# HKUST-KnowComp/DummyNode4GraphLearning

Measured on AMD Instinct MI355X. Metric: edges/sec fwd+bwd on dummy-augmented RGIN conv, higher is better.
Workload: dtype bf16; 1 GPU; config5: RGINLayer(256,256,R=16,basis,relu) fwd+bwd, ONE global batch of 32768 graphs cut by parallel.shard_graphs over 1 GPU(s) (rank 0: N=1015808, E=3997696), SI dummy augmentation; global_edges=3997696, parallelism=dp1, rows_P=3112960, grad_bucket_bytes=2491904, hip_graph=True, sub_batches=1

## Files before the change

### dummynode4graphlearning_amd/_lib.py

```python
import ctypes
import os

import torch

_HERE = os.path.dirname(os.path.abspath(__file__))
LIB_PATH = os.environ.get("DN_HIP_LIB") or os.path.join(_HERE, "libdn_hip.so")

c_i32, c_i64, c_f32, c_sz = ctypes.c_int32, ctypes.c_int64, ctypes.c_float, ctypes.c_size_t
P = ctypes.c_void_p

class WgradJob(ctypes.Structure):
    _fields_ = [("A", P), ("A2", P), ("idx_a", P), ("G", P), ("G2", P), ("idx_g", P), ("mask_a_bits", P), ("na1", c_i32), ("ng1", c_i32),
                ("colsum_of", c_i32), ("first_rel", c_i32), ("row0", c_i32), ("act_slope", c_f32)]


_SIGS = {
    "dn_version": (ctypes.c_int, []),
    "dn_last_error": (ctypes.c_char_p, []),
    "dn_runtime_probe": (ctypes.c_int, [P]),
    "dn_gather_segsum_f32": (ctypes.c_int, [P, c_i64, c_i32, P, P, P, c_i64, c_i64, P, P, c_f32, c_i32, P]),
    "dn_gather_segsum_bf16": (ctypes.c_int, [P, c_i64, c_i32, P, P, P, c_i64, c_i64, P, P, c_f32, c_i32, P]),
    "dn_segment_sum_f32": (ctypes.c_int, [P, c_i32, P, c_i64, P, P]),
    "dn_segment_sum_bf16": (ctypes.c_int, [P, c_i32, P, c_i64, P, P]),
    "dn_segment_mean_f32": (ctypes.c_int, [P, c_i32, P, c_i64, P, P]),
# ... 25 lines not shown
    "dn_row_index_workspace_bytes": (c_sz, [c_i64, c_i64, c_i64]),
    "dn_row_index_build_i32": (ctypes.c_int, [c_i64, c_i64, c_i64, P, P, P, c_i32, c_f32] + [P] * 10 +
                               [ctypes.POINTER(c_i64), ctypes.POINTER(c_i32), ctypes.POINTER(c_i32), P, c_sz, P]),
    "dn_row_index_local_workspace_bytes": (c_sz, [c_i64, c_i64, c_i64, c_i64]),
    "dn_row_index_build_local_i32": (ctypes.c_int, [c_i64, c_i64, c_i64, c_i64, P, P, P, P, P, c_i32, c_f32] + [P] * 10 +
                                     [ctypes.POINTER(c_i64), ctypes.POINTER(c_i32), ctypes.POINTER(c_i32),
                                      ctypes.POINTER(c_i32), P, P, P, P, P, ctypes.POINTER(c_i32), P, c_sz, P]),
    "dn_rows_wgrad_multi_bf16": (ctypes.c_int, [ctypes.POINTER(WgradJob), c_i32, c_i32, c_i64, P, c_i64, P, P, c_i32, P, P, P, c_sz, P]),
    "dn_rows_wgrad_multi_f32": (ctypes.c_int, [ctypes.POINTER(WgradJob), c_i32, c_i32, c_i64, P, c_i64, P, P, P, P, c_sz, P]),
    "dn_rows_chain2_f32": (ctypes.c_int, [P, c_i32, P, P, c_i32, P, P, P, P, c_i32, c_i64, P, P, c_i32, c_f32, P, P, P]),
    "dn_layer_graphs_fwd_bf16": (ctypes.c_int, [P, c_i32, P, P, P, c_i32, P, P, P, P, c_f32, P, P, P, P, P, c_i64, c_i64, P, P, P, P, P, P, P,
                                                P, P, P]),
    "dn_layer_graphs_bwd_bf16": (ctypes.c_int, [P, c_i32, P, P, c_i32, P, P, c_f32, P, P, P, P, P, P, P, c_i64, c_i64, P, P, P, P, P, P, P,
                                                P]),
    "dn_conv_graphs_max_nodes": (c_i32, []),
    "dn_conv_graphs_max_edges": (c_i32, []),
    "dn_conv_graphs_bf16": (ctypes.c_int, [P, c_i32, P, c_i32, P, P, c_i32, P, P, P, P, P, c_i64, c_i64, P, P, P, P, P, P]),
    "dn_conv_index_workspace_bytes": (c_sz, [c_i64, c_i64, c_i64, c_i64, c_i32, c_i64]),
    "dn_conv_index_build_i32": (ctypes.c_int, [c_i64, c_i64, c_i64, c_i64, P, P, P, P, P, c_i32, c_f32] + [P] * 10 +
                                [ctypes.POINTER(c_i64), ctypes.POINTER(c_i32), ctypes.POINTER(c_i32),
                                 ctypes.POINTER(c_i32), P, P, P, P, P, ctypes.POINTER(c_i32)] +
                                [c_i32, c_i32, c_i64] + [P] * 8 + [c_i32, c_i64] + [P] * 8 + [c_i32, c_i32, P, P] + [c_i32, c_i32, c_i64, P, P] +
                                [ctypes.POINTER(c_i32), P, c_sz, P]),
    "dn_row_tables_build_i32": (ctypes.c_int, [c_i32, P, c_i32, c_i64, P, P, ctypes.c_uint64, P]),
    "dn_sweep_tables_build_i32": (ctypes.c_int, [c_i32, P, P, P, c_i64, c_i32, c_i32, ctypes.c_uint64, P, P, P]),
    "dn_slot_table_build_i32": (ctypes.c_int, [c_i64, c_i32, c_i32, P, P, c_i32, c_i32, P, P, P, P]),
    "dn_fold_tables_build_async_i32": (ctypes.c_int, [c_i64, c_i64, P, P, P, P, P, P, c_sz, P]),
    "dn_rows_wgrad_workspace_bytes": (c_sz, [c_i64, c_i32, c_i32]),
    "dn_rows_wgrad_bf16": (ctypes.c_int, [P, P, c_i32, P, P, P, c_i32, P, c_i32, c_i32, c_i64, P, c_i64, P, P, c_i32,
                                          c_i32, P, P, P, P, P, c_f32, P, c_sz, P]),
    "dn_rows_transform_bf16": (ctypes.c_int, [P, P, c_i32, P, c_i32, c_i32, P, P, c_i32, P, P, c_i64, P, c_i32, c_f32, P]),
    "dn_relu_bwd_bf16": (ctypes.c_int, [P, P, P, c_i64, c_f32, P]),
    "dn_rows_chain2_bf16": (ctypes.c_int, [P, c_i32, P, P, c_i32, P, P, P, P, c_i32, c_i64, P, P, P, P, c_i32, c_f32, P]),
    "dn_rows_selfsum_bf16": (ctypes.c_int, [P, c_i32, P, P, P, P, c_i32, P, c_i32, c_i64, P, P, P, c_i32, P, P, c_i32, c_i32, c_i32, P]),
    "dn_overflow_rows_add_bf16": (ctypes.c_int, [P, c_i32, P, c_i32, c_i64, P, P, c_i32, c_i32, c_i32, P, P]),
    "dn_close_units_capacity": (c_i64, [c_i64, c_i64, c_i32]),
    "dn_close_units_workspace_bytes": (c_sz, [c_i64, c_i32]),
    "dn_close_units_build_i32": (ctypes.c_int, [c_i64, c_i32, c_i32, P, c_i64, c_i32, c_i32, P, P, c_i64, c_i32, c_i32, P, P, P, c_i64, P,
                                                P, P, P, c_i32, P, c_sz, P]),
    "dn_fold_graph_tiles_build_i32": (ctypes.c_int, [c_i64, c_i64, P, P, P, P, P, P, P]),
    "dn_fold_graph_tiles_multi_capacity": (c_i64, [c_i64, c_i32]),
    "dn_fold_graph_tiles_multi_build_i32": (ctypes.c_int, [c_i64, c_i64, P, P, P, c_i32, P, P, P, P, c_i64, P, P]),
    "dn_rows_close_bf16": (ctypes.c_int, [P, c_i32, P, c_i32, P, P, P, P, c_i32, P, P, c_i64, P, P, P, P, P, P, P]),
    "dn_bdd_compose": (ctypes.c_int, [P, c_i64, c_i32, c_i32, c_i32, c_i32, P, P]),
    "dn_bdd_extract": (ctypes.c_int, [P, c_i64, c_i32, c_i32, c_i32, c_i32, P, P]),
    "dn_fold_tables_workspace_bytes": (c_sz, [c_i64]),
    "dn_fold_tables_build_i32": (ctypes.c_int, [c_i64, c_i64, P, P, P, P, ctypes.POINTER(ctypes.c_int32), P, c_sz, P]),
    "dn_fold_tail_bf16": (ctypes.c_int, [P, P, c_i64, c_i32, P, P, P, P, c_i32, P]),
    "dn_rows_transform_f32": (ctypes.c_int, [P, P, c_i32, P, c_i32, c_i32, P, P, c_i32, P, P, c_i64, P, c_i32, c_f32, P, c_i32, c_i32, c_i32, P]),
    "dn_rows_wgrad_f32": (ctypes.c_int, [P, P, c_i32, P, P, P, c_i32, P, c_i32, c_i32, c_i64, P, c_i64, P, P, c_i32, P, P, P,
                                         c_i32, c_f32, P, c_sz, P]),
    "dn_relu_bwd_f32": (ctypes.c_int, [P, P, P, c_i64, c_f32, P]),
    "dn_rows_gemm_f32": (ctypes.c_int, [P, P, P, c_i32, c_i32, c_i32, P, c_i64, P, P]),
    "dn_rows_gemm_bf16": (ctypes.c_int, [P, P, P, c_i32, c_i32, c_i32, P, c_i64, P, P]),
    "dn_rows_wgrad_any_workspace_bytes": (c_sz, [c_i64, c_i32, c_i32]),
    "dn_rows_wgrad_any_f32": (ctypes.c_int, [P, P, c_i32, c_i32, c_i64, P, c_i64, P, P, P, P, c_sz, P]),
    "dn_rows_wgrad_any_bf16": (ctypes.c_int, [P, P, c_i32, c_i32, c_i64, P, c_i64, P, P, P, P, c_sz, P]),
    "dn_batchnorm_rows_workspace_bytes": (c_sz, [c_i64, c_i32]),
    "dn_batchnorm_rows_f32": (ctypes.c_int, [P, c_i64, c_i32, P, P, c_f32, P, P, P, P, P, P, c_f32, c_i32, P, P, c_sz, P]),
    "dn_batchnorm_rows_bf16": (ctypes.c_int, [P, c_i64, c_i32, P, P, c_f32, P, P, P, P, P, P, c_f32, c_i32, P, P, c_sz, P]),
    "dn_batchnorm_rows_bwd_f32": (ctypes.c_int, [P, P, c_i64, c_i32, P, P, P, P, c_i32, P, P, P, P, c_sz, P]),
    "dn_batchnorm_rows_bwd_bf16": (ctypes.c_int, [P, P, c_i64, c_i32, P, P, P, P, c_i32, P, P, P, P, c_sz, P]),
    "dn_edge_norm_f32": (ctypes.c_int, [c_i32, c_i32, c_i64, c_i64] + [P] * 7 + [P]),
    "dn_degrees_i32": (ctypes.c_int, [c_i64, c_i64, P, P, P, P, P]),
    "dn_si_filter_meta_f32": (ctypes.c_int, [c_i64, P, P, P, c_i64, P, P, P, c_i64, c_i32, c_i32, c_i32, c_i32, P, P, P]),
    "dn_si_filter_meta_bf16": (ctypes.c_int, [c_i64, P, P, P, c_i64, P, P, P, c_i64, c_i32, c_i32, c_i32, c_i32, P, P, P]),
# ... 116 lines not shown
```

### dummynode4graphlearning_amd/csrc/build.py

```python
import hashlib
import os
import subprocess
import sys
from concurrent.futures import ThreadPoolExecutor

HERE = os.path.dirname(os.path.abspath(__file__))
PKG = os.path.dirname(HERE)
ROOT = os.path.dirname(PKG)
SOURCES = ["dn_runtime.hip", "dn_segment.hip", "dn_index.hip", "dn_index_local.hip", "dn_conv_index.hip", "dn_graphsum.hip", "dn_rel.hip", "dn_rel_ring.hip", "dn_close.hip", "dn_conv_graph.hip", "dn_chain2.hip", "dn_weights.hip", "dn_rel_f32.hip", "dn_gemm.hip", "dn_norm.hip", "dn_simodel.hip", "dn_dual.hip"]
HEADERS = ["dn_common.h", "dn_internal.h", os.path.join(ROOT, "include", "dn_hip.h")]
LIB = os.path.join(PKG, "libdn_hip.so")
OBJDIR = os.path.join(HERE, "_obj")
ARCH = "gfx950"
FLAGS = ["-O3", "-std=c++17", "-fPIC", "--offload-arch=" + ARCH, "-fno-gpu-rdc", "-Wno-unused-result",
         "-I" + os.path.join(ROOT, "include")]


def _hipcc():
    for c in (os.environ.get("HIPCC"), "/opt/rocm/bin/hipcc", "hipcc"):
        if c and (os.path.isabs(c) and os.path.exists(c) or not os.path.isabs(c)):
            return c
    raise RuntimeError("hipcc not found")


def _digest(paths):
    h = hashlib.sha256()
    for p in paths:
        with open(p, "rb") as f:
            h.update(f.read())
    h.update(" ".join(FLAGS).encode())
    return h.hexdigest()


def build(force=False, verbose=True, tuning=False):
    global FLAGS
    if (tuning or os.environ.get("DN_BUILD_TUNING") == "1") and "-DDN_TUNING_ENV" not in FLAGS:
        FLAGS = FLAGS + ["-DDN_TUNING_ENV"]
    for extra in os.environ.get("DN_BUILD_EXTRA", "").split():
        if extra not in FLAGS:
            FLAGS = FLAGS + [extra]
    srcs = [os.path.join(HERE, s) for s in SOURCES if os.path.exists(os.path.join(HERE, s))]
    hdrs = [h if os.path.isabs(h) else os.path.join(HERE, h) for h in HEADERS]
# ... 37 lines not shown
```

### dummynode4graphlearning_amd/csrc/dn_internal.h

```cpp
#pragma once
#include <hip/hip_runtime.h>
#include <stdint.h>

namespace dn_internal {

int launch_transform_ring256(const void* X, const void* X2, int32_t n1, const int32_t* idx, const void* Wn, const void* bias,
                             int32_t relu, int32_t nt_store, const void* mask_pos, const int32_t* tiles, int64_t num_tiles,
                             int64_t tiles_per_wg, void* Y, int32_t w_kn, float slope, hipStream_t st);

bool chain2_ring_supported(bool has_mask0, bool has_mask1, bool has_bits1, bool has_bits2);
int launch_chain2_ring256(const void* X, const void* W1n, const void* b1, const void* W2n, const void* b2, int32_t flags,
                          const void* mask0, const void* mask1, int64_t N, void* Y1, void* Y2, void* bits1, void* bits2,
                          float slope, hipStream_t st);

constexpr int kRilPlanWords = 14;

int ril_queue(int64_t G, int64_t N, int64_t R, int64_t E, const int32_t* node_ptr, const int32_t* edge_ptr, const int32_t* src,
              const int32_t* dst, const int32_t* etype, int32_t self_loop, float edge_frac, int32_t* row_in, int32_t* row_out,
              int32_t* aux_f_ptr, int32_t* aux_f_idx, int32_t* aux_b_ptr, int32_t* aux_b_idx, int32_t* dst_ptr, int32_t* dst_rows,
              int32_t* src_ptr, int32_t* src_rows, int32_t* rel_ptr_dev, int32_t* tile_ptr_f, int32_t* fold_info_f,
              int32_t* tile_ptr_b, int32_t* fold_info_b, bool verdicts, bool plan, void* workspace, size_t workspace_bytes,
              int32_t** meta_dev, hipStream_t st);
void ril_unpack(const int32_t* h_meta, int64_t R, int64_t* host_counts, int32_t* host_rel_ptr, int32_t* host_modes,
                int32_t* host_status, int32_t* host_absorb);

struct CloseUnitsDir {
    const int32_t *tile_ptr, *list_ptr, *list_rows;
    int32_t num_edge_rows, drop_beg, drop_end;
    const int32_t *drop_enable, *dyn;
    int32_t *unit_ptr, *units, *ent_row;
    uint32_t* ent_mask;
    const int32_t *chunk_tile = nullptr, *chunk_graph = nullptr;
    int32_t chunks_per_wg = 0;
    const int32_t* tile_ptr_alt = nullptr;
};
struct FoldMultiDir {
    const int32_t *seg_ptr, *seg_nodes, *add_idx;
    int32_t *chunk_tile, *chunk_graph, *tile_ptr, *fold_info, *dev_ok;
    const int32_t* gate;
};
int fold_multi_queue(int64_t N, int64_t num_segments, int nd, const FoldMultiDir* dirs, int32_t num_chunks, int64_t tile_capacity,
                     bool with_valid, hipStream_t st);
int close_units_queue(int64_t N, int32_t num_wg, int64_t num_tiles, int32_t agg_units, int32_t xcd_order, int64_t num_list_entries,
                      int64_t unit_capacity, int nd, const CloseUnitsDir* dirs, void* workspace, size_t workspace_bytes, hipStream_t st,
                      int32_t alt_order, int64_t alt_num_tiles);

// ... 6 lines not shown
```

### dummynode4graphlearning_amd/csrc/dn_rel.hip

```cpp
#include <cstdlib>

#include "dn_common.h"
#include "dn_internal.h"
#include "../../include/dn_hip.h"

namespace {

typedef __bf16 bf16_t;
typedef short short4v __attribute__((ext_vector_type(4)));
typedef short short8v __attribute__((ext_vector_type(8)));
typedef bf16_t bf16x8 __attribute__((ext_vector_type(8)));
typedef float f32x4 __attribute__((ext_vector_type(4)));

constexpr int kWgThreads = 512;
constexpr int kTileRows = 64;
constexpr int kPad = 8;

struct Chunk {
    int32_t rel, beg, end, pad;
};

__device__ __forceinline__ int32_t colsum_for(int32_t colsum_arg, int32_t rel) {
    const int32_t only = colsum_arg >> 8;
    return (only == 0 || rel + 1 == only) ? (colsum_arg & 0xff) : 0;
// ... 1821 lines not shown
        *reinterpret_cast<bf16x8*>(bufX + pr * SX + pc * 8) = xr;
        if (j < n) *reinterpret_cast<bf16x8*>(aux + (size_t)j * H + pc * 8) = xr;
        __syncthreads();
        f32x4 acc[MT];
#pragma unroll
        for (int m = 0; m < MT; ++m) acc[m] = f32x4{0.f, 0.f, 0.f, 0.f};
#pragma unroll
        for (int ks = 0; ks < KS; ++ks) {
#pragma unroll
            for (int m = 0; m < MT; ++m) {
                const bf16x8 xf = *reinterpret_cast<const bf16x8*>(bufX + (m * 16 + (lane & 15)) * SX + ks * 32 + 8 * (lane >> 4));
                acc[m] = __builtin_amdgcn_mfma_f32_16x16x32_bf16(wf[ks], xf, acc[m], 0, 0, 0);
            }
        }
#pragma unroll
        for (int m = 0; m < MT; ++m)
            *reinterpret_cast<f32x4*>(bufY + (m * 16 + (lane & 15)) * SYF + n0 + 4 * (lane >> 4)) = acc[m];
        __syncthreads();
        if (j < n) {
            const float4 y0 = *reinterpret_cast<const float4*>(bufY + pr * SYF + pc * 8);
            const float4 y1 = *reinterpret_cast<const float4*>(bufY + pr * SYF + pc * 8 + 4);
            const float y[8] = {y0.x, y0.y, y0.z, y0.w, y1.x, y1.y, y1.z, y1.w};
            const uint32_t w[4] = {cur.x, cur.y, cur.z, cur.w};
            bf16x8 o;
#pragma unroll
            for (int i = 0; i < 4; ++i) {
                o[2 * i] = (bf16_t)(__uint_as_float(w[i] << 16) + y[2 * i]);
                o[2 * i + 1] = (bf16_t)(__uint_as_float(w[i] & 0xffff0000u) + y[2 * i + 1]);
            }
            *reinterpret_cast<bf16x8*>(out + (size_t)orow * H + pc * 8) = o;
        }
        __syncthreads();
    }
}

}

extern "C" {

int dn_fold_tail_bf16(const float* part, const int32_t* part_ptr, int64_t num_segments, int32_t H, const void* Wn,
                      const int32_t* idx, void* aux, void* out, int32_t w_kn, dn_stream_t stream) {
    DN_REQUIRE(num_segments >= 0 && num_segments < INT32_MAX, "dn_fold_tail: bad sizes");
    DN_REQUIRE(H == 64 || H == 128 || H == 256, "dn_fold_tail: H must be 64, 128 or 256");
    if (num_segments == 0) return DN_OK;
    DN_REQUIRE(part && part_ptr && Wn && idx && aux && out, "dn_fold_tail: NULL pointer");
    DN_REQUIRE((reinterpret_cast<uintptr_t>(part) | reinterpret_cast<uintptr_t>(Wn) | reinterpret_cast<uintptr_t>(aux) |
                reinterpret_cast<uintptr_t>(out)) % 16 == 0, "dn_fold_tail: unaligned pointer");
    const int32_t num_tiles = (int32_t)dn_cdiv(num_segments, kSsRows);
    const unsigned grid = (unsigned)(num_tiles < 512 ? num_tiles : 512);
    hipStream_t st = (hipStream_t)stream;
    const float* p = part;
    const bf16_t *w = (const bf16_t*)Wn;
    bf16_t *a = (bf16_t*)aux, *o = (bf16_t*)out;
    const int32_t n = (int32_t)num_segments;
    if (H == 256) hipLaunchKernelGGL((fold_tail_kernel<256>), dim3(grid), dim3(1024), 0, st, p, part_ptr, w, idx, n, num_tiles, a, o, w_kn);
    else if (H == 128) hipLaunchKernelGGL((fold_tail_kernel<128>), dim3(grid), dim3(512), 0, st, p, part_ptr, w, idx, n, num_tiles, a, o, w_kn);
    else hipLaunchKernelGGL((fold_tail_kernel<64>), dim3(grid), dim3(256), 0, st, p, part_ptr, w, idx, n, num_tiles, a, o, w_kn);
    DN_CHECK_LAUNCH();
    return DN_OK;
}

int dn_relu_bwd_bf16(const void* g, const void* y, void* out, int64_t numel, float act_slope, dn_stream_t stream) {
    DN_REQUIRE(numel >= 0 && numel % 8 == 0, "dn_relu_bwd: numel must be a non-negative multiple of 8");
    if (numel == 0) return DN_OK;
    DN_REQUIRE(g && y && out, "dn_relu_bwd: NULL pointer");
    DN_REQUIRE((reinterpret_cast<uintptr_t>(g) | reinterpret_cast<uintptr_t>(y) | reinterpret_cast<uintptr_t>(out)) % 16 == 0,
// ... 205 lines not shown
```

### dummynode4graphlearning_amd/ops.py

```python
import ctypes
import os as _os
import threading as _threading

import torch

from . import _lib
from ._lib import check, lib, ptr, require_gpu, stream_ptr

I32 = torch.int32


class KernelTimer:

    def __init__(self):
        self.records = []
        self.enabled = True

    def launch(self, tag, fn):
        if not self.enabled:
            return fn()
        a, b = torch.cuda.Event(enable_timing=True), torch.cuda.Event(enable_timing=True)
        a.record()
        r = fn()
        b.record()
# ... 1889 lines not shown

    @staticmethod
    def _backward(ctx, g):
        x, weight, y = ctx.saved_tensors
        g = g.contiguous()
        tiles, chunks = _dense_table(x.shape[0], x.device)
        gx = gw = gb = None
        need_w = ctx.needs_input_grad[1] or (ctx.has_bias and ctx.needs_input_grad[2])
        if ctx.relu and not need_w:
            g = relu_bwd(g, y)
        if need_w:
            gm = torch.empty_like(g) if ctx.relu else None
            with f32_exact(ctx.exact_w):
                gw, cs = rows_wgrad(g, x, chunks, 1, out_dtype=weight.dtype, colsum_of=1, mask_a=y if ctx.relu else None,
                                    a_out=gm)
            g = gm if ctx.relu else g
            gw = gw[0]
            if ctx.has_bias:
                gb = cs[0].to(g.dtype)
        if ctx.needs_input_grad[0]:
            kn = g.dtype == torch.float32
            gx = rows_transform(g, (weight if kn else weight.t()).contiguous().unsqueeze(0), tiles, x.shape[0], w_kn=kn)
        return gx, gw, gb, None


def relu_bwd(g, y, slope=0.0):
    require_gpu(g, y)
    out = torch.empty_like(g)
    fn = lib().dn_relu_bwd_f32 if g.dtype == torch.float32 else lib().dn_relu_bwd_bf16
    check(fn(ptr(g), ptr(y), ptr(out), g.numel(), float(slope), stream_ptr()), "dn_relu_bwd")
    return out


class _ReluMlpFn(torch.autograd.Function):

    @staticmethod
    def forward(ctx, x, slope, *wb):
        ctx.f32_mode = f32_mode()
        n = len(wb) // 2
        x = x.contiguous()
        ctx.slope = slope = float(slope)
        if n == 2 and CHAIN2_ENABLED and x.dtype == torch.bfloat16:
            h1, h2, bits1, bits2 = rows_chain2(x, wb[0], wb[1], True, wb[2], wb[3], True, want_bits=True, slope=slope)
            ctx.n, ctx.chain = n, True
            ctx.has_bias = [wb[1] is not None, wb[3] is not None]
            ctx.save_for_backward(x, h1, bits1, bits2, wb[0], wb[2])
            return h2
        if (n == 2 and CHAIN2_F32_ENABLED and x.dtype == torch.float32 and x.shape[1] in (64, 128) and not f32_mode()
                and all(t is None or t.dtype == torch.float32 for t in wb)):
            h1, h2 = rows_chain2_f32(x, wb[0], wb[1], True, wb[2], wb[3], True, slope=slope)
            ctx.n, ctx.chain = n, "f32"
            ctx.has_bias = [wb[1] is not None, wb[3] is not None]
            ctx.save_for_backward(x, h1, h2, wb[0], wb[2])
            return h2
        tiles, _ = _dense_table(x.shape[0], x.device)
        acts = [x]
        for i in range(n):
            w, b = wb[2 * i], wb[2 * i + 1]
            acts.append(rows_transform(acts[-1], w.contiguous().unsqueeze(0), tiles, x.shape[0],
                                       bias=None if b is None else b.contiguous().view(1, -1), relu=True, slope=slope))
        ctx.n, ctx.chain = n, False
        ctx.has_bias = [wb[2 * i + 1] is not None for i in range(n)]
        ctx.save_for_backward(*acts, *[wb[2 * i] for i in range(n)])
        return acts[-1]

    @staticmethod
    @_backward_in_forward_mode
    def backward(ctx, gout):
        n, slope = ctx.n, ctx.slope
        saved = ctx.saved_tensors
        g = gout.contiguous()
        grads = [None] * (2 + 2 * n)
        if ctx.chain == "f32":
            x0, h1, h2, w1, w2 = saved
            _, chunks = _dense_table(x0.shape[0], x0.device)
            gw2, cs2 = rows_wgrad(g, h1, chunks, 1, out_dtype=w2.dtype, colsum_of=1, mask_a=h2, slope=slope)
            g1, g0 = rows_chain2_f32(g, w2, None, False, w1, None, False, mask0=h2, mask1=h1, w_kn=(True, True), slope=slope)
            gw1, cs1 = rows_wgrad(g1, x0, chunks, 1, out_dtype=w1.dtype, colsum_of=1)
            grads[2], grads[4] = gw1[0], gw2[0]
            if ctx.has_bias[0]:
                grads[3] = cs1[0].to(g.dtype)
            if ctx.has_bias[1]:
                grads[5] = cs2[0].to(g.dtype)
            grads[0] = g0 if ctx.needs_input_grad[0] else None
            return tuple(grads)
        if ctx.chain:
            x0, h1, bits1, bits2, w1, w2 = saved
            _, chunks = _dense_table(x0.shape[0], x0.device)
            gw2, cs2 = rows_wgrad(g, h1, chunks, 1, out_dtype=w2.dtype, colsum_of=1, mask_a_bits=bits2, colsum_lp=True, slope=slope)
            g1, g0 = rows_chain2(g, w2, None, False, w1, None, False, mask0_bits=bits2, mask1_bits=bits1, w_kn=(True, True),
                                 slope=slope)
            gw1, cs1 = rows_wgrad(g1, x0, chunks, 1, out_dtype=w1.dtype, colsum_of=1, colsum_lp=True)
            grads[2], grads[4] = gw1[0], gw2[0]
            if ctx.has_bias[0]:
                grads[3] = cs1[0].to(g.dtype)
            if ctx.has_bias[1]:
                grads[5] = cs2[0].to(g.dtype)
            grads[0] = g0 if ctx.needs_input_grad[0] else None
            return tuple(grads)
        acts, ws = saved[:n + 1], saved[n + 1:]
        tiles, chunks = _dense_table(acts[0].shape[0], acts[0].device)
        for i in range(n - 1, -1, -1):
            w = ws[i]
            if i == n - 1:
                gm = torch.empty_like(g)
                gw, cs = rows_wgrad(g, acts[i], chunks, 1, out_dtype=w.dtype, colsum_of=1, mask_a=acts[n], a_out=gm, slope=slope)
                g = gm
            else:
                gw, cs = rows_wgrad(g, acts[i], chunks, 1, out_dtype=w.dtype, colsum_of=1)
            grads[2 + 2 * i] = gw[0]
            if ctx.has_bias[i]:
                grads[3 + 2 * i] = cs[0].to(g.dtype)
            if i > 0 or ctx.needs_input_grad[0]:
                kn = g.dtype == torch.float32
                g = rows_transform(g, (w if kn else w.t()).contiguous().unsqueeze(0), tiles, g.shape[0],
                                   mask_pos=acts[i] if i > 0 else None, slope=slope, w_kn=kn)
        grads[0] = g if ctx.needs_input_grad[0] else None
        return tuple(grads)


LAYER_GRAPHS_ENABLED = _os.environ.get("DN_LAYER_GRAPHS", "1") != "0"
# ... 858 lines not shown
```

### include/dn_hip.h

```cpp
#ifndef DN_HIP_H
#define DN_HIP_H

#include <stddef.h>
#include <stdint.h>

#ifdef __cplusplus
extern "C" {
#endif

#define DN_OK 0
#define DN_ERR_ARG (-1)
#define DN_ERR_HIP (-2)
#define DN_ERR_WORKSPACE (-3)
#define DN_ERR_UNSUPPORTED (-4)

typedef void* dn_stream_t;

int dn_version(void);
const char* dn_last_error(void);
int dn_runtime_probe(const void* device_ptr);

int dn_gather_segsum_f32(const float* in, int64_t in_rows, int32_t H, const int32_t* idx,
                         const float* scale, const int32_t* ptr, int64_t S, int64_t M, float* out,
                         const float* self_in, float self_coef, int32_t mean, dn_stream_t stream);
// ... 195 lines not shown
                             dn_stream_t stream);
int64_t dn_fold_graph_tiles_multi_capacity(int64_t N, int32_t num_chunks);
int dn_fold_graph_tiles_multi_build_i32(int64_t N, int64_t num_segments, const int32_t* seg_ptr, const int32_t* seg_nodes,
                                        const int32_t* add_idx, int32_t num_chunks, int32_t* chunk_tile, int32_t* chunk_graph,
                                        int32_t* tile_ptr, int32_t* fold_info, int64_t tile_capacity, int32_t* dev_ok,
                                        dn_stream_t stream);
int dn_fold_graph_tiles_build_i32(int64_t N, int64_t num_segments, const int32_t* seg_ptr, const int32_t* seg_nodes,
                                  const int32_t* add_idx, int32_t* tile_ptr, int32_t* fold_info, int32_t* dev_ok,
                                  dn_stream_t stream);
int dn_rows_close_bf16(const void* X, int32_t H, const void* W, int32_t w_kn, const void* bias, const void* S,
                       const int32_t* unit_ptr, const int32_t* units, int32_t num_wg, const int32_t* ent_row,
                       const uint32_t* ent_mask, int64_t N, void* out, const int32_t* fold_info, float* seg_part,
                       const void* W_agg, void* aux, const int32_t* agg_idx, dn_stream_t stream);

size_t dn_fold_tables_workspace_bytes(int64_t num_segments);
int dn_fold_tables_build_i32(int64_t N, int64_t num_segments, const int32_t* seg_ptr, const int32_t* seg_nodes,
                             int32_t* fold_info, int32_t* part_ptr, int32_t* host_ok, void* workspace, size_t workspace_bytes,
                             dn_stream_t stream);
int dn_fold_tables_build_async_i32(int64_t N, int64_t num_segments, const int32_t* seg_ptr, const int32_t* seg_nodes,
                                   int32_t* fold_info, int32_t* part_ptr, int32_t* dev_ok, void* workspace,
                                   size_t workspace_bytes, dn_stream_t stream);

int dn_fold_tail_bf16(const float* part, const int32_t* part_ptr, int64_t num_segments, int32_t H, const void* Wn,
                      const int32_t* idx, void* aux, void* out, int32_t w_kn, dn_stream_t stream);

int dn_bdd_compose(const void* blocks, int64_t R, int32_t B, int32_t si, int32_t so, int32_t elem_bytes, void* dense,
                   dn_stream_t stream);
int dn_bdd_extract(const void* dense, int64_t R, int32_t B, int32_t si, int32_t so, int32_t elem_bytes, void* blocks,
                   dn_stream_t stream);

int dn_rows_chain2_bf16(const void* X, int32_t H, const void* W1n, const void* b1, int32_t relu1, const void* mask0_bits,
                        const void* mask1_bits, const void* W2n, const void* b2, int32_t relu2, int64_t N, void* Y1, void* Y2,
                        void* bits1, void* bits2, int32_t w_kn, float act_slope, dn_stream_t stream);

int dn_relu_bwd_bf16(const void* g, const void* y, void* out, int64_t numel, float act_slope, dn_stream_t stream);

int dn_rows_transform_f32(const float* X, const float* X2, int32_t n1, const int32_t* idx, int32_t Hi, int32_t Ho,
                          const float* Wn, const float* bias, int32_t relu, const float* mask_pos,
                          const int32_t* tiles, int64_t num_tiles, float* Y, int32_t precision, float act_slope,
                          const float* W_loop, int32_t loop_rel, int32_t bias_rel, int32_t w_kn, dn_stream_t stream);
int dn_rows_wgrad_f32(const float* A, const float* A2, int32_t na1, const int32_t* idx_a, const float* G,
                      const float* G2, int32_t ng1, const int32_t* idx_g, int32_t Hi, int32_t Ho, int64_t R,
                      const int32_t* chunks, int64_t num_chunks, const int32_t* chunk_ptr, float* out,
                      int32_t colsum_of, float* out_colsum, const float* mask_a, float* a_out, int32_t precision,
                      float act_slope, void* workspace, size_t workspace_bytes, dn_stream_t stream);
int dn_relu_bwd_f32(const float* g, const float* y, float* out, int64_t numel, float act_slope, dn_stream_t stream);

int dn_rows_gemm_f32(const float* A, const float* W, const float* bias, int32_t K, int32_t N, int32_t transposed, const int32_t* tiles,
                     int64_t num_tiles, float* Y, dn_stream_t stream);
int dn_rows_gemm_bf16(const void* A, const void* W, const void* bias, int32_t K, int32_t N, int32_t transposed, const int32_t* tiles,
                      int64_t num_tiles, void* Y, dn_stream_t stream);
size_t dn_rows_wgrad_any_workspace_bytes(int64_t num_chunks, int32_t K, int32_t N);
int dn_rows_wgrad_any_f32(const float* A, const float* G, int32_t K, int32_t N, int64_t R, const int32_t* chunks, int64_t num_chunks,
                          const int32_t* chunk_ptr, float* out, float* colsum_out, void* workspace, size_t workspace_bytes,
                          dn_stream_t stream);
int dn_rows_wgrad_any_bf16(const void* A, const void* G, int32_t K, int32_t N, int64_t R, const int32_t* chunks, int64_t num_chunks,
                           const int32_t* chunk_ptr, void* out, float* colsum_out, void* workspace, size_t workspace_bytes,
                           dn_stream_t stream);

size_t dn_batchnorm_rows_workspace_bytes(int64_t N, int32_t C);
int dn_batchnorm_rows_f32(const float* X, int64_t N, int32_t C, const float* weight, const float* bias, float eps, float* Y, float* mean,
                          float* var, float* rstd, float* running_mean, float* running_var, float momentum, int32_t relu,
                          int64_t* num_batches_tracked, void* workspace, size_t workspace_bytes, dn_stream_t stream);
int dn_batchnorm_rows_bf16(const void* X, int64_t N, int32_t C, const float* weight, const float* bias, float eps, void* Y, float* mean,
                           float* var, float* rstd, float* running_mean, float* running_var, float momentum, int32_t relu,
                           int64_t* num_batches_tracked, void* workspace, size_t workspace_bytes, dn_stream_t stream);
// ... 103 lines not shown
```

Baseline: 1.321 billion edges/s.

## Fuse RGIN MLP backward weight-grad, bias colsum and data-grad into one kernel

```diff
diff --git a/dummynode4graphlearning_amd/_lib.py b/dummynode4graphlearning_amd/_lib.py
--- a/dummynode4graphlearning_amd/_lib.py
+++ b/dummynode4graphlearning_amd/_lib.py
@@ -81,6 +81,7 @@
     "dn_rows_transform_bf16": (ctypes.c_int, [P, P, c_i32, P, c_i32, c_i32, P, P, c_i32, P, P, c_i64, P, c_i32, c_f32, P]),
     "dn_relu_bwd_bf16": (ctypes.c_int, [P, P, P, c_i64, c_f32, P]),
     "dn_rows_chain2_bf16": (ctypes.c_int, [P, c_i32, P, P, c_i32, P, P, P, P, c_i32, c_i64, P, P, P, P, c_i32, c_f32, P]),
+    "dn_mlp_bwd_fused_bf16": (ctypes.c_int, [P, P, P, P, P, c_i64, c_i32, P, c_i64, P, P, c_i32, P, P, P, c_f32, P, c_sz, P]),
     "dn_rows_selfsum_bf16": (ctypes.c_int, [P, c_i32, P, P, P, P, c_i32, P, c_i32, c_i64, P, P, P, c_i32, P, P, c_i32, c_i32, c_i32, P]),
     "dn_overflow_rows_add_bf16": (ctypes.c_int, [P, c_i32, P, c_i32, c_i64, P, P, c_i32, c_i32, c_i32, P, P]),
     "dn_close_units_capacity": (c_i64, [c_i64, c_i64, c_i32]),
diff --git a/dummynode4graphlearning_amd/csrc/build.py b/dummynode4graphlearning_amd/csrc/build.py
--- a/dummynode4graphlearning_amd/csrc/build.py
+++ b/dummynode4graphlearning_amd/csrc/build.py
@@ -7,7 +7,7 @@
 HERE = os.path.dirname(os.path.abspath(__file__))
 PKG = os.path.dirname(HERE)
 ROOT = os.path.dirname(PKG)
-SOURCES = ["dn_runtime.hip", "dn_segment.hip", "dn_index.hip", "dn_index_local.hip", "dn_conv_index.hip", "dn_graphsum.hip", "dn_rel.hip", "dn_rel_ring.hip", "dn_close.hip", "dn_conv_graph.hip", "dn_chain2.hip", "dn_weights.hip", "dn_rel_f32.hip", "dn_gemm.hip", "dn_norm.hip", "dn_simodel.hip", "dn_dual.hip"]
+SOURCES = ["dn_runtime.hip", "dn_segment.hip", "dn_index.hip", "dn_index_local.hip", "dn_conv_index.hip", "dn_graphsum.hip", "dn_rel.hip", "dn_rel_ring.hip", "dn_close.hip", "dn_conv_graph.hip", "dn_chain2.hip", "dn_mlp_bwd.hip", "dn_weights.hip", "dn_rel_f32.hip", "dn_gemm.hip", "dn_norm.hip", "dn_simodel.hip", "dn_dual.hip"]
 HEADERS = ["dn_common.h", "dn_internal.h", os.path.join(ROOT, "include", "dn_hip.h")]
 LIB = os.path.join(PKG, "libdn_hip.so")
 OBJDIR = os.path.join(HERE, "_obj")
diff --git a/dummynode4graphlearning_amd/csrc/dn_internal.h b/dummynode4graphlearning_amd/csrc/dn_internal.h
--- a/dummynode4graphlearning_amd/csrc/dn_internal.h
+++ b/dummynode4graphlearning_amd/csrc/dn_internal.h
@@ -12,6 +12,9 @@
 int launch_chain2_ring256(const void* X, const void* W1n, const void* b1, const void* W2n, const void* b2, int32_t flags,
                           const void* mask0, const void* mask1, int64_t N, void* Y1, void* Y2, void* bits1, void* bits2,
                           float slope, hipStream_t st);
+
+int launch_wgrad_reduce(const float* workspace, const int32_t* chunk_ptr, int64_t num_chunks, int32_t H, int64_t R, void* out,
+                        int32_t out_is_f32, bool with_colsum, float* out_colsum, void* out_colsum_lp, hipStream_t st);
 
 constexpr int kRilPlanWords = 14;
 
diff --git a/dummynode4graphlearning_amd/csrc/dn_mlp_bwd.hip b/dummynode4graphlearning_amd/csrc/dn_mlp_bwd.hip
--- /dev/null
+++ b/dummynode4graphlearning_amd/csrc/dn_mlp_bwd.hip
@@ -0,0 +1,361 @@
+#include "dn_common.h"
+#include "dn_internal.h"
+#include "../../include/dn_hip.h"
+
+namespace {
+
+typedef __bf16 bf16_t;
+typedef short short4v __attribute__((ext_vector_type(4)));
+typedef short short8v __attribute__((ext_vector_type(8)));
+typedef bf16_t bf16x8 __attribute__((ext_vector_type(8)));
+typedef float f32x4 __attribute__((ext_vector_type(4)));
+typedef unsigned int u32x4 __attribute__((ext_vector_type(4)));
+
+struct Chunk {
+    int32_t rel, beg, end, pad;
+};
+
+constexpr int kH = 256;
+constexpr int kRowB = 2 * kH;
+constexpr int kTR = 32;
+constexpr int kMatB = kTR * kRowB;
+constexpr int kBitsB = kTR * (kH / 8);
+constexpr int kStB = 2 * kMatB + 2 * kBitsB;
+constexpr int kNST = 4;
+constexpr int kThreads = 512;
+constexpr int kDma = 4, kST = 2;
+static_assert(kStB % 1024 == 0, "the fragment addressing XORs low bits of stage-relative offsets");
+
+__device__ __attribute__((aligned(16))) uint4 g_mb_zero[64];
+__device__ __attribute__((aligned(16))) uint4 g_mb_dump[64 * 8];
+
+__device__ __forceinline__ int swz(int r) {
+    return ((r >> 2) & 1) | ((r & 3) << 1) | ((((r >> 3) ^ (r >> 2)) & 1) << 3);
+}
+
+__device__ __forceinline__ uint32_t pack2(float a, float b) {
+    typedef bf16_t bf16x2 __attribute__((ext_vector_type(2)));
+    bf16x2 v;
+    v[0] = (bf16_t)a;
+    v[1] = (bf16_t)b;
+    return __builtin_bit_cast(uint32_t, v);
+}
+
+template <bool MASKED>
+__device__ __forceinline__ void mb_wait(int t) {
+    if constexpr (MASKED) {
+        if (t == 0) { wait_vmcnt<2 + kDma>(); return; }
+        if (t == 1) { wait_vmcnt<2 + kDma + kST>(); return; }
+        wait_vmcnt<2 + kDma + 2 * kST>();
+    } else {
+        if (t == 0) { wait_vmcnt<2 * kDma>(); return; }
+        if (t == 1) { wait_vmcnt<2 * kDma + kST>(); return; }
+        if (t == 2) { wait_vmcnt<2 * kDma + 2 * kST>(); return; }
+        wait_vmcnt<2 * kDma + 3 * kST>();
+    }
+}
+
+struct Frag {
+    short4v lo, hi;
+};
+__device__ __forceinline__ bf16x8 frag_val(const Frag& f) {
+    const short8v v = {f.lo[0], f.lo[1], f.lo[2], f.lo[3], f.hi[0], f.hi[1], f.hi[2], f.hi[3]};
+    return __builtin_bit_cast(bf16x8, v);
+}
+#define DN_MB_TR(fr, ad, ad2)                                                                                          \
+    do {                                                                                                              \
+        asm volatile("ds_read_b64_tr_b16 %0, %1" : "=v"((fr).lo) : "v"(ad));                                          \
+        asm volatile("ds_read_b64_tr_b16 %0, %1 offset:2048" : "=v"((fr).hi) : "v"(ad2));                             \
+    } while (0)
+#define DN_MB_READ128(dst, addr, OFF) asm volatile("ds_read_b128 %0, %1 offset:" #OFF : "=v"(dst) : "v"(addr))
+static_assert(4 * kRowB == 2048, "offset of a transposed fragment's second half");
+
+template <bool MASKED>
+__global__ __launch_bounds__(kThreads) void mlp_bwd_fused_kernel(const bf16_t* __restrict__ G, const bf16_t* __restrict__ A,
+                                                                 const bf16_t* __restrict__ Wkn,
+                                                                 const uint8_t* __restrict__ bits_in,
+                                                                 const uint8_t* __restrict__ bits_out, int32_t N,
+                                                                 const Chunk* __restrict__ chunks, float* __restrict__ partial,
+                                                                 float* __restrict__ colsum_partial, bf16_t* __restrict__ Gn,
+                                                                 float slope) {
+    __shared__ __attribute__((aligned(1024))) char lds[kNST * kStB];
+    typedef __attribute__((address_space(3))) char* lds_wp;
+    const unsigned lds_base = (unsigned)(uintptr_t)(lds_wp)lds;
+    const int tid = threadIdx.x, lane = tid & 63;
+    const int wave = __builtin_amdgcn_readfirstlane(tid >> 6);
+    const Chunk ch = chunks[blockIdx.x];
+    const int32_t cbeg = max(ch.beg, 0), cend = min(ch.end, N);
+    const int ntiles = cend > cbeg ? (cend - cbeg + kTR - 1) / kTR : 0;
+    if (ntiles <= 0) {
+        for (int i = tid; i < kH * kH; i += kThreads) partial[(size_t)blockIdx.x * kH * kH + i] = 0.f;
+        if (tid < kH) colsum_partial[(size_t)blockIdx.x * kH + tid] = 0.f;
+        return;
+    }
+
+    bf16x8 wf[8][2];
+    dn_load_w_kn32<8>(Wkn, kH, 32 * wave, lane, lds + wave * 2048, wf);
+    wait_vmcnt<0>();
+#pragma unroll
+    for (int ks = 0; ks < 8; ++ks)
+#pragma unroll
+        for (int n = 0; n < 2; ++n) asm volatile("" : "+v"(wf[ks][n]));
+    __syncthreads();
+
+    auto fresh = [&]() __attribute__((always_inline)) {
+        int l = lane;
+        asm volatile("" : "+v"(l));
+        return l;
+    };
+    const char* zero = reinterpret_cast<const char*>(g_mb_zero);
+    auto issue = [&](int T) __attribute__((always_inline)) {
+        const int ln = fresh(), rin = ln >> 5, cpos = ln & 31;
+        const unsigned st = lds_base + (unsigned)(T % kNST) * kStB;
+        const int64_t r0 = (int64_t)cbeg + (int64_t)T * kTR;
+        uint64_t pas[2];
+#pragma unroll
+        for (int jj = 0; jj < 2; ++jj) {
+            const int rl = 4 * wave + 2 * jj + rin;
+            const uint64_t gch = (uint64_t)((cpos ^ swz(rl)) << 4);
+            const int64_t p = r0 + rl;
+            const bool ok = p < (int64_t)cend;
+            const uint64_t off = (uint64_t)p * kRowB + gch, z = (uint64_t)(uintptr_t)zero + gch;
+            const uint64_t pg = ok ? (uint64_t)(uintptr_t)G + off : z;
+            pas[jj] = ok ? (uint64_t)(uintptr_t)A + off : z;
+            glds16(reinterpret_cast<const char*>(pg), st + (unsigned)(4 * wave + 2 * jj) * kRowB);
+        }
+        if constexpr (MASKED) {
+            const int64_t p = r0 + (ln >> 1);
+            const size_t boff = (size_t)p * (kH / 8) + (size_t)(ln & 1) * 16;
+            const bool ok = p < (int64_t)cend;
+            if (wave == (T & 7)) glds16(ok ? reinterpret_cast<const char*>(bits_in) + boff : zero + ln * 16, st + 2 * kMatB);
+            if (wave == ((T + 4) & 7))
+                glds16(ok ? reinterpret_cast<const char*>(bits_out) + boff : zero + ln * 16, st + 2 * kMatB + kBitsB);
+        }
+#pragma unroll
+        for (int jj = 0; jj < 2; ++jj)
+            glds16(reinterpret_cast<const char*>(pas[jj]), st + (unsigned)kMatB + (unsigned)(4 * wave + 2 * jj) * kRowB);
+    };
+
+    float cs[8] = {0.f, 0.f, 0.f, 0.f, 0.f, 0.f, 0.f, 0.f};
+    auto add_cs = [&](const uint4& v) __attribute__((always_inline)) {
+        const uint32_t w[4] = {v.x, v.y, v.z, v.w};
+#pragma unroll
+        for (int i = 0; i < 4; ++i) {
+            cs[2 * i] += __uint_as_float(w[i] << 16);
+            cs[2 * i + 1] += __uint_as_float(w[i] & 0xffff0000u);
+        }
+    };
+    auto mask_tile = [&](int T) __attribute__((always_inline)) {
+        const int ln = fresh(), mrow = 2 * wave + (ln >> 5), mq = ln & 31, mchunk = mq ^ swz(mrow);
+        char* sT = lds + (T % kNST) * kStB;
+        const uint8_t* sB = reinterpret_cast<const uint8_t*>(sT + 2 * kMatB);
+#pragma unroll
+        for (int jj = 0; jj < 2; ++jj) {
+            const int r = mrow + 16 * jj;
+            u32x4* pp = reinterpret_cast<u32x4*>(sT + r * kRowB + mq * 16);
+            const int32_t kb = (int32_t)sB[r * (kH / 8) + mchunk];
+            u32x4 v = *pp;
+#pragma unroll
+            for (int i = 0; i < 4; ++i) {
+                const uint32_t m0 = (uint32_t)__builtin_amdgcn_sbfe(kb, 2 * i, 1), m1 = (uint32_t)__builtin_amdgcn_sbfe(kb, 2 * i + 1, 1);
+                const uint32_t mk = (m0 & 0xffffu) | (m1 & 0xffff0000u);
+                uint32_t alt = 0u;
+                if (slope != 0.f) alt = pack2(__uint_as_float(v[i] << 16) * slope, __uint_as_float(v[i] & 0xffff0000u) * slope);
+                v[i] = (v[i] & mk) | (alt & ~mk);
+            }
+            *pp = v;
+            add_cs(make_uint4(v[0], v[1], v[2], v[3]));
+        }
+    };
+    auto colsum_tile = [&](int T) __attribute__((always_inline)) {
+        const int ln = fresh(), mrow = 2 * wave + (ln >> 5), mq = ln & 31;
+        const char* sT = lds + (T % kNST) * kStB;
+#pragma unroll
+        for (int jj = 0; jj < 2; ++jj) add_cs(*reinterpret_cast<const uint4*>(sT + (mrow + 16 * jj) * kRowB + mq * 16));
+    };
+
+    const int wm = wave >> 2, wn = wave & 3;
+    f32x4 acc[8][4];
+#pragma unroll
+    for (int m = 0; m < 8; ++m)
+#pragma unroll
+        for (int n = 0; n < 4; ++n) acc[m][n] = f32x4{0.f, 0.f, 0.f, 0.f};
+    auto tr_lane = [&](int ln, int piece0) __attribute__((always_inline)) {
+        const int fg = ln >> 4, fq = (ln & 15) >> 2, fp = ln & 3, fR = 8 * fg + fq;
+        return lds_base + (unsigned)(fR * kRowB + (((piece0 + (fp >> 1)) ^ swz(fR)) << 4) + 8 * (fp & 1));
+    };
+
+    f32x4 dacc[2];
+    bf16x8 xf[4];
+
+#define DN_MB_FETCH(SLOT, KS, HH)                                                                                     \
+    {                                                                                                                 \
+        const unsigned a_ = (sg + off0) ^ (unsigned)(((KS) & 3) << 6);                                                \
+        if ((HH) == 0) {                                                                                              \
+            if ((KS) < 4) { DN_MB_READ128(xf[SLOT], a_, 0); } else { DN_MB_READ128(xf[SLOT], a_, 256); }              \
+        } else {                                                                                                      \
+            if ((KS) < 4) { DN_MB_READ128(xf[SLOT], a_, 8192); } else { DN_MB_READ128(xf[SLOT], a_, 8448); }          \
+        }                                                                                                             \
+    }
+#define DN_MB_MFMA2(SLOT, KS)                                                                                         \
+    _Pragma("unroll") for (int n = 0; n < 2; ++n)                                                                      \
+        dacc[n] = __builtin_amdgcn_mfma_f32_16x16x32_bf16(wf[KS][n], xf[SLOT], dacc[n], 0, 0, 0);                    \
+    __builtin_amdgcn_sched_barrier(0);
+#define DN_MB_KSTEP(SLOT, KS, CNT)                                                                                    \
+    asm volatile("s_waitcnt lgkmcnt(" #CNT ")" : "+v"(xf[SLOT]));                                                     \
+    DN_MB_MFMA2(SLOT, KS)
+#define DN_MB_DGRAD_HALF(HH)                                                                                          \
+    {                                                                                                                 \
+        DN_MB_FETCH(0, 0, HH) DN_MB_FETCH(1, 1, HH) DN_MB_FETCH(2, 2, HH) DN_MB_FETCH(3, 3, HH)                       \
+        __builtin_amdgcn_sched_barrier(0);                                                                            \
+        asm volatile("s_waitcnt lgkmcnt(3)" : "+v"(xf[0]));                                                           \
+        _Pragma("unroll") for (int n = 0; n < 2; ++n)                                                                  \
+            dacc[n] = __builtin_amdgcn_mfma_f32_16x16x32_bf16(wf[0][n], xf[0], f32x4{0.f, 0.f, 0.f, 0.f}, 0, 0, 0);  \
+        __builtin_amdgcn_sched_barrier(0);                                                                            \
+        DN_MB_FETCH(0, 4, HH) __builtin_amdgcn_sched_barrier(0);                                                      \
+        DN_MB_KSTEP(1, 1, 3) DN_MB_FETCH(1, 5, HH) __builtin_amdgcn_sched_barrier(0);                                 \
+        DN_MB_KSTEP(2, 2, 3) DN_MB_FETCH(2, 6, HH) __builtin_amdgcn_sched_barrier(0);                                 \
+        DN_MB_KSTEP(3, 3, 3) DN_MB_FETCH(3, 7, HH) __builtin_amdgcn_sched_barrier(0);                                 \
+        DN_MB_KSTEP(0, 4, 3)                                                                                          \
+        DN_MB_KSTEP(1, 5, 2)                                                                                          \
+        DN_MB_KSTEP(2, 6, 1)                                                                                          \
+        DN_MB_KSTEP(3, 7, 0)                                                                                          \
+        const int64_t p = r0 + 16 * (HH);                                                                             \
+        float v[8];                                                                                                   \
+        _Pragma("unroll") for (int n = 0; n < 2; ++n)                                                                  \
+        _Pragma("unroll") for (int i = 0; i < 4; ++i) v[4 * n + i] = dacc[n][i];                                       \
+        if constexpr (MASKED) {                                                                                       \
+            const int32_t kb = (int32_t)sB1[(16 * (HH) + j) * (kH / 8) + bcol];                                       \
+            _Pragma("unroll") for (int i = 0; i < 8; ++i) {                                                            \
+                const uint32_t mk = (uint32_t)__builtin_amdgcn_sbfe(kb, i, 1);                                        \
+                const uint32_t alt = slope != 0.f ? __float_as_uint(v[i] * slope) : 0u;                               \
+                v[i] = __uint_as_float((__float_as_uint(v[i]) & mk) | (alt & ~mk));                                   \
+            }                                                                                                         \
+        }                                                                                                             \
+        u32x4 o;                                                                                                      \
+        _Pragma("unroll") for (int i = 0; i < 4; ++i) o[i] = pack2(v[2 * i], v[2 * i + 1]);                            \
+        char* dst = p < (int64_t)cend ? reinterpret_cast<char*>(Gn) + (uint64_t)p * kRowB + ycol : dump;              \
+        __builtin_nontemporal_store(o, reinterpret_cast<u32x4*>(dst));   \
+        __builtin_amdgcn_sched_barrier(0);                                                                            \
+    }
+
+#pragma unroll 1
+    for (int T = 0; T < kNST - 1; ++T) issue(T);
+    if constexpr (MASKED) {
+        wait_vmcnt<2 + 2 * kDma>();
+        __builtin_amdgcn_s_barrier();
+        mask_tile(0);
+    }
+
+#pragma unroll 1
+    for (int t = 0; t < ntiles; ++t) {
+        mb_wait<MASKED>(t);
+        asm volatile("s_waitcnt lgkmcnt(0)" ::: "memory");
+        __builtin_amdgcn_s_barrier();
+        issue(t + kNST - 1);
+        const unsigned sg = (unsigned)(t % kNST) * kStB;
+        __builtin_amdgcn_sched_barrier(0);
+        {
+            const int ln = fresh();
+            const unsigned va = tr_lane(ln, 16 * wm) + sg, vb = tr_lane(ln, 8 * wn) + (unsigned)kMatB + sg, va2 = va ^ 0x90u, vb2 = vb ^ 0x90u;
+            Frag fb[4], fa[2];
+#pragma unroll
+            for (int n = 0; n < 4; ++n) DN_MB_TR(fb[n], vb ^ (unsigned)(n << 5), vb2 ^ (unsigned)(n << 5));
+#pragma unroll
+            for (int m = 0; m < 2; ++m) DN_MB_TR(fa[m], va ^ (unsigned)(m << 5), va2 ^ (unsigned)(m << 5));
+#pragma unroll
+            for (int m = 0; m < 8; ++m) {
+                Frag& f = fa[m & 1];
+                if (m == 0)
+                    asm volatile("s_waitcnt lgkmcnt(2)" : "+v"(f.lo), "+v"(f.hi), "+v"(fb[0].lo), "+v"(fb[0].hi), "+v"(fb[1].lo), "+v"(fb[1].hi),
+                                 "+v"(fb[2].lo), "+v"(fb[2].hi), "+v"(fb[3].lo), "+v"(fb[3].hi));
+                else if (m < 7) asm volatile("s_waitcnt lgkmcnt(2)" : "+v"(f.lo), "+v"(f.hi));
+                else asm volatile("s_waitcnt lgkmcnt(0)" : "+v"(f.lo), "+v"(f.hi));
+                const bf16x8 av = frag_val(f);
+#pragma unroll
+                for (int n = 0; n < 4; ++n) acc[m][n] = __builtin_amdgcn_mfma_f32_16x16x32_bf16(av, frag_val(fb[n]), acc[m][n], 0, 0, 0);
+                if (m + 2 < 8) DN_MB_TR(f, va ^ (unsigned)((m + 2) << 5), va2 ^ (unsigned)((m + 2) << 5));
+                __builtin_amdgcn_sched_barrier(0);
+            }
+        }
+        {
+            const int ln = fresh(), j = ln & 15, g = ln >> 4;
+            const unsigned off0 = lds_base + (unsigned)(j * kRowB + ((g ^ swz(j)) << 4));
+            char* dump = reinterpret_cast<char*>(g_mb_dump) + wave * 1024 + ln * 16;
+            const unsigned ycol = (unsigned)(32 * wave + 8 * g) * 2;
+            const unsigned bcol = (unsigned)(4 * wave + g);
+            const uint8_t* sB1 = reinterpret_cast<const uint8_t*>(lds + (t % kNST) * kStB + 2 * kMatB + kBitsB);
+            const int64_t r0 = (int64_t)cbeg + (int64_t)t * kTR + j;
+            DN_MB_DGRAD_HALF(0)
+            DN_MB_DGRAD_HALF(1)
+        }
+        if constexpr (MASKED) mask_tile(t + 1);
+        else colsum_tile(t);
+    }
+#undef DN_MB_DGRAD_HALF
+#undef DN_MB_MFMA2
+#undef DN_MB_KSTEP
+#undef DN_MB_FETCH
+    wait_vmcnt<0>();
+    asm volatile("s_waitcnt lgkmcnt(0)" ::: "memory");
+    __builtin_amdgcn_s_barrier();
+
+    float* out = partial + (size_t)blockIdx.x * kH * kH;
+    const int k0 = wm * (kH / 2), n0 = wn * (kH / 4);
+#pragma unroll
+    for (int m = 0; m < 8; ++m)
+#pragma unroll
+        for (int n = 0; n < 4; ++n)
+#pragma unroll
+            for (int i = 0; i < 4; ++i) {
+                const int k = k0 + m * 16 + (lane >> 4) * 4 + i, c = n0 + n * 16 + (lane & 15);
+                out[(size_t)k * kH + c] = acc[m][n][i];
+            }
+    const int mrow = tid >> 5, mchunk = (tid & 31) ^ swz(mrow);
+    float* red = reinterpret_cast<float*>(lds);
+#pragma unroll
+    for (int i = 0; i < 8; ++i) red[mrow * kH + mchunk * 8 + i] = cs[i];
+    __syncthreads();
+    if (tid < kH) {
+        float sum = 0.f;
+        for (int sl = 0; sl < kThreads / 32; ++sl) sum += red[sl * kH + tid];
+        colsum_partial[(size_t)blockIdx.x * kH + tid] = sum;
+    }
+}
+#undef DN_MB_TR
+#undef DN_MB_READ128
+
+}
+
+extern "C" int dn_mlp_bwd_fused_bf16(const void* G, const void* A, const void* W_kn, const void* mask_in_bits,
+                                     const void* mask_out_bits, int64_t N, int32_t H, const int32_t* chunks, int64_t num_chunks,
+                                     const int32_t* chunk_ptr, void* out_w, int32_t out_is_f32, float* out_colsum,
+                                     void* out_colsum_lp, void* g_next, float act_slope, void* workspace, size_t workspace_bytes,
+                                     dn_stream_t stream) {
+    DN_REQUIRE(H == 256, "dn_mlp_bwd_fused: unsupported width %d (256 only)", H);
+    DN_REQUIRE(N >= 0 && N < 0x7fffffffLL && num_chunks >= 0, "dn_mlp_bwd_fused: bad sizes");
+    DN_REQUIRE((mask_in_bits == nullptr) == (mask_out_bits == nullptr), "dn_mlp_bwd_fused: both masks or neither");
+    DN_REQUIRE(out_w && chunk_ptr && out_colsum, "dn_mlp_bwd_fused: NULL pointer");
+    DN_REQUIRE(num_chunks == 0 || (G && A && W_kn && chunks && workspace && g_next), "dn_mlp_bwd_fused: NULL pointer");
+    DN_REQUIRE(workspace_bytes >= (size_t)num_chunks * ((size_t)H * H + H) * sizeof(float), "dn_mlp_bwd_fused: workspace too small");
+    DN_REQUIRE((reinterpret_cast<uintptr_t>(G) | reinterpret_cast<uintptr_t>(A) | reinterpret_cast<uintptr_t>(W_kn) |
+                reinterpret_cast<uintptr_t>(mask_in_bits) | reinterpret_cast<uintptr_t>(mask_out_bits) |
+                reinterpret_cast<uintptr_t>(g_next) | reinterpret_cast<uintptr_t>(workspace) |
+                reinterpret_cast<uintptr_t>(out_colsum)) % 16 == 0, "dn_mlp_bwd_fused: unaligned pointer");
+    hipStream_t st = (hipStream_t)stream;
+    float* ws = (float*)workspace;
+    if (num_chunks > 0) {
+        float* csp = ws + (size_t)num_chunks * H * H;
+        const Chunk* ch = reinterpret_cast<const Chunk*>(chunks);
+        if (mask_in_bits)
+            hipLaunchKernelGGL((mlp_bwd_fused_kernel<true>), dim3((unsigned)num_chunks), dim3(kThreads), 0, st, (const bf16_t*)G,
+                               (const bf16_t*)A, (const bf16_t*)W_kn, (const uint8_t*)mask_in_bits, (const uint8_t*)mask_out_bits,
+                               (int32_t)N, ch, ws, csp, (bf16_t*)g_next, act_slope);
+        else
+            hipLaunchKernelGGL((mlp_bwd_fused_kernel<false>), dim3((unsigned)num_chunks), dim3(kThreads), 0, st, (const bf16_t*)G,
+                               (const bf16_t*)A, (const bf16_t*)W_kn, (const uint8_t*)nullptr, (const uint8_t*)nullptr, (int32_t)N, ch,
+                               ws, csp, (bf16_t*)g_next, act_slope);
+        DN_CHECK_LAUNCH();
+    }
+    return dn_internal::launch_wgrad_reduce(ws, chunk_ptr, num_chunks, H, 1, out_w, out_is_f32, true, out_colsum, out_colsum_lp, st);
+}
diff --git a/dummynode4graphlearning_amd/csrc/dn_rel.hip b/dummynode4graphlearning_amd/csrc/dn_rel.hip
--- a/dummynode4graphlearning_amd/csrc/dn_rel.hip
+++ b/dummynode4graphlearning_amd/csrc/dn_rel.hip
@@ -1877,6 +1877,25 @@
         }
         __syncthreads();
     }
+}
+
+}
+
+namespace dn_internal {
+
+int launch_wgrad_reduce(const float* workspace, const int32_t* chunk_ptr, int64_t num_chunks, int32_t H, int64_t R, void* out,
+                        int32_t out_is_f32, bool with_colsum, float* out_colsum, void* out_colsum_lp, hipStream_t st) {
+    const int64_t tile = (int64_t)H * H;
+    const float* csp = with_colsum ? workspace + (size_t)num_chunks * tile : nullptr;
+    dim3 grid((unsigned)(dn_cdiv(tile, 128) + (csp ? dn_cdiv(H, 128) : 0)), (unsigned)R);
+    if (out_is_f32)
+        hipLaunchKernelGGL((wgrad_reduce_kernel<float>), grid, dim3(256), 0, st, workspace, chunk_ptr, tile, (float*)out, csp, H,
+                           out_colsum, (float*)out_colsum_lp);
+    else
+        hipLaunchKernelGGL((wgrad_reduce_kernel<bf16_t>), grid, dim3(256), 0, st, workspace, chunk_ptr, tile, (bf16_t*)out, csp, H,
+                           out_colsum, (bf16_t*)out_colsum_lp);
+    DN_CHECK_LAUNCH();
+    return DN_OK;
 }
 
 }
diff --git a/dummynode4graphlearning_amd/ops.py b/dummynode4graphlearning_amd/ops.py
--- a/dummynode4graphlearning_amd/ops.py
+++ b/dummynode4graphlearning_amd/ops.py
@@ -1945,6 +1945,41 @@
     return out
 
 
+MLP_BWD_FUSED_ENABLED = _os.environ.get("DN_MLP_BWD_FUSED", "1") != "0"
+MLP_BWD_FUSED_MIN_ROWS = int(_os.environ.get("DN_MLP_BWD_FUSED_MIN_ROWS", str(1 << 18)))
+
+
+def mlp_bwd_fused_supported(g, a, w):
+    return (g.dtype == torch.bfloat16 and a.dtype == torch.bfloat16 and w.dtype == torch.bfloat16 and g.dim() == 2
+            and g.shape[0] > 0 and g.shape[1] == 256 and a.shape == g.shape and tuple(w.shape) == (256, 256))
+
+
+def mlp_bwd_fused(g, a, w, chunk_table, mask_in_bits=None, mask_out_bits=None, slope=0.0):
+    chunks, chunk_ptr, nchunks = chunk_table
+    g, a, w = g.contiguous(), a.contiguous(), w.contiguous()
+    require_gpu(g, a, w, chunks, chunk_ptr, mask_in_bits, mask_out_bits)
+    assert mlp_bwd_fused_supported(g, a, w) and nchunks > 0
+    N, H = g.shape
+    assert (mask_in_bits is None) == (mask_out_bits is None)
+    for m in (mask_in_bits, mask_out_bits):
+        assert m is None or (m.dtype == torch.uint8 and m.shape == (N, H // 8) and m.is_contiguous())
+    gw = torch.empty((H, H), dtype=w.dtype, device=g.device)
+    colsum = torch.empty((H,), dtype=torch.float32, device=g.device)
+    gb = torch.empty((H,), dtype=w.dtype, device=g.device)
+    g_next = torch.empty_like(g)
+    ws = _ws(lib().dn_rows_wgrad_workspace_bytes(nchunks, H, H), g.device)
+
+    def _launch():
+        check(lib().dn_mlp_bwd_fused_bf16(ptr(g), ptr(a), ptr(w), ptr(mask_in_bits), ptr(mask_out_bits), N, H, ptr(chunks), nchunks,
+                                          ptr(chunk_ptr), ptr(gw), 0, ptr(colsum), ptr(gb), ptr(g_next), float(slope), ptr(ws),
+                                          ws.numel(), stream_ptr()), "dn_mlp_bwd_fused_bf16")
+    if kernel_timer is not None:
+        kernel_timer.launch("mlp_bwd_fused", _launch)
+    else:
+        _launch()
+    return gw, gb, g_next
+
+
 class _ReluMlpFn(torch.autograd.Function):
 
     @staticmethod
@@ -2000,6 +2035,21 @@
         if ctx.chain:
             x0, h1, bits1, bits2, w1, w2 = saved
             _, chunks = _dense_table(x0.shape[0], x0.device)
+            if (MLP_BWD_FUSED_ENABLED and x0.shape[0] >= MLP_BWD_FUSED_MIN_ROWS and mlp_bwd_fused_supported(g, h1, w2)
+                    and mlp_bwd_fused_supported(g, x0, w1)):
+                gw2, gb2, g1 = mlp_bwd_fused(g, h1, w2, chunks, mask_in_bits=bits2, mask_out_bits=bits1, slope=slope)
+                if ctx.needs_input_grad[0]:
+                    gw1, gb1, g0 = mlp_bwd_fused(g1, x0, w1, chunks, slope=slope)
+                else:
+                    gw1, cs1 = rows_wgrad(g1, x0, chunks, 1, out_dtype=w1.dtype, colsum_of=1, colsum_lp=True)
+                    gw1, gb1, g0 = gw1[0], cs1[0], None
+                grads[2], grads[4] = gw1, gw2
+                if ctx.has_bias[0]:
+                    grads[3] = gb1.to(g.dtype)
+                if ctx.has_bias[1]:
+                    grads[5] = gb2.to(g.dtype)
+                grads[0] = g0
+                return tuple(grads)
             gw2, cs2 = rows_wgrad(g, h1, chunks, 1, out_dtype=w2.dtype, colsum_of=1, mask_a_bits=bits2, colsum_lp=True, slope=slope)
             g1, g0 = rows_chain2(g, w2, None, False, w1, None, False, mask0_bits=bits2, mask1_bits=bits1, w_kn=(True, True),
                                  slope=slope)
diff --git a/include/dn_hip.h b/include/dn_hip.h
--- a/include/dn_hip.h
+++ b/include/dn_hip.h
@@ -251,6 +251,11 @@
 int dn_rows_chain2_bf16(const void* X, int32_t H, const void* W1n, const void* b1, int32_t relu1, const void* mask0_bits,
                         const void* mask1_bits, const void* W2n, const void* b2, int32_t relu2, int64_t N, void* Y1, void* Y2,
                         void* bits1, void* bits2, int32_t w_kn, float act_slope, dn_stream_t stream);
+
+int dn_mlp_bwd_fused_bf16(const void* G, const void* A, const void* W_kn, const void* mask_in_bits, const void* mask_out_bits,
+                          int64_t N, int32_t H, const int32_t* chunks, int64_t num_chunks, const int32_t* chunk_ptr, void* out_w,
+                          int32_t out_is_f32, float* out_colsum, void* out_colsum_lp, void* g_next, float act_slope,
+                          void* workspace, size_t workspace_bytes, dn_stream_t stream);
 
 int dn_relu_bwd_bf16(const void* g, const void* y, void* out, int64_t numel, float act_slope, dn_stream_t stream);
 
```

Result: faster. 1.357 billion edges/s, median of 6 (+2.8%).
